# ebarnett2/batotp

Measured on AMD Instinct MI355X. Metric: constraint-evaluated waypoints/sec + traversal-time err vs CPU ref, higher is better.
Workload: dtype f64

## Files before the change

batotp_amd/csrc/batotp_hip.hip:

```cpp
#include <hip/hip_runtime.h>

#include <algorithm>
#include <cmath>
#include <cstdio>
#include <cstdlib>
#include <cstring>
#include <new>
#include <thread>
#include <type_traits>
#include <vector>

#include "batotp_hip.h"
#include "batotp_models.h"
#include "kernels.hip.h"
#include "sweep1.hip.h"
#include "sweep8.hip.h"
#include "pointwise_va.hip.h"
#include "spline_stream.hip.h"
#include "spline_tile.hip.h"
#include "spline_lanes.hip.h"
#include "resample.hip.h"
#include "output.hip.h"

static inline unsigned seriesBlock(int64_t series)
{
   const int64_t lanes = (series + 255) / 256;
   return (unsigned)(lanes < 4 ? 4 : (lanes > 64 ? 64 : lanes));
}

static inline bool seriesLanesPay(int64_t series) { return series <= 4096; }

using namespace bk;

constexpr int BATOTP_CERT_HOLD_DEFAULT = 3;

static thread_local char g_err[512] = "";

static int hipFail(hipError_t e, const char *what)
{
   snprintf(g_err, sizeof(g_err), "%s: %s", what, hipGetErrorString(e));
   return BATOTP_ERR_HIP;
}
#define HIP_TRY(call)                                              \
   do                                                              \
   {                                                               \
      hipError_t e_ = (call);                                      \
      if (e_ != hipSuccess) return hipFail(e_, #call);             \
   } while (0)

extern "C" const char *batotp_hip_last_error(void) { return g_err; }

#define BK_STR2(x) #x
#define BK_STR(x) BK_STR2(x)
static const char kBuiltWith[] = "clang " __clang_version__ " / HIP " BK_STR(HIP_VERSION_MAJOR) "." BK_STR(HIP_VERSION_MINOR) "." BK_STR(HIP_VERSION_PATCH);
static const char kFlatValidatedWith[] =
   "clang 22.0.0git (https://github.com/RadeonOpenCompute/llvm-project roc-7.2.0 26014 7b800a19466229b8479a78de19143dc33c3ab9b5) / HIP 7.2.26015";

extern "C" int batotp_hip_toolchain(char *built_with, char *validated_with, int32_t cap)
{
   if (cap < 1) return BATOTP_ERR_ARG;
   if (built_with) { strncpy(built_with, kBuiltWith, (size_t)cap - 1); built_with[cap - 1] = 0; }
   if (validated_with) { strncpy(validated_with, kFlatValidatedWith, (size_t)cap - 1); validated_with[cap - 1] = 0; }
   return BATOTP_OK;
}

struct Arena
{
   void *p = nullptr;
   size_t cap = 0;
};

struct batotp_ctx
{
   Arena ws[4];
   std::vector<double> kinTheta, kinTrig;
   Arena xfer;
   uint64_t rsEpoch = 0;
   int device = 0;
   hipStream_t stream = nullptr;
   hipStream_t stream2 = nullptr;
   hipEvent_t evJoin = nullptr;
   int overlap = 0;
   int sweepGroup = 0;
   int pathsPerWave = 0;
   int sweepTouch[2] = {-1, -1};
   int sweepHold[2] = {-2, -2};
   int splineTiles = -1;
   int flatForm = 1;
   int fastForward = 1;
   int certHold = -1;
   int poison = 0;
   int rsTrace = 0;
   uint64_t rsTraceSums[8] = {0, 0, 0, 0, 0, 0, 0, 0};
   unsigned long long *dTrace = nullptr;
   std::vector<double> rsTraceData[8];
   int64_t rsBudget = 0, outBudget = 0;
   int pathOrder = 1;
   int k3Form = 1;
   int flatStatus = 0;
   char builtWith[192] = "";
};

struct SweepPlan
{
   int feat = 0;
   bool uni = false;
   int lanes = 0;
   int ppw = 0;
   int hold = -1, touch = 0, ff = 0, holdc = 0;
   bool flat = false;
   bool form8 = false;
   int ff1 = 0;
};

struct batotp_batch
{
   batotp_ctx *ctx = nullptr;
   batotp_problem prob;
   DevProblem P;
   int32_t B = 0;
   int64_t cap = 0;
   int64_t totalKnots = 0;
   std::vector<PathInfo> pinfo;
   bool needPar = false;
   bool k3Pending = false;
   bool compact = false;
   bool pairsAll = false;
   int kmC = 0;
   bool kinDone = false, dynDone = false, sitesSet = false, revDone = false, trigSet = false;
   bool inPlace = false;
   bool revGone = false;
   bool mvcInCurves = false, mvcValid = false;
   bool revStale = false, fwdStale = false;

   DevProblem *dP = nullptr;
   PathInfo *dPinfo = nullptr;
   double *dY = nullptr, *dSC = nullptr, *dCoef = nullptr, *dSamp = nullptr, *dDyn = nullptr, *dTrig = nullptr, *dMvc = nullptr;
   double2 *dRev = nullptr, *dFwd = nullptr;
   batotp_path_result *dRes = nullptr;
   int *dOrder = nullptr;
   double *dProf = nullptr;
   double *dStage = nullptr;
   int *dSink = nullptr;
   double *dElim = nullptr;
   double *dKM = nullptr;
   batotp_serial_model *dModel = nullptr;
   batotp_serial_model hModel;
   double *dJTrig = nullptr;
   bool hasSerial = false, jtrigSet = false;
   int *dTileOff = nullptr, *dDirty = nullptr;
   double *dEdge = nullptr;
   int totalTiles = 0, nchMax = 0, lastTileNch = 0;
   double *dUp = nullptr;
   int64_t upDoubles = 0;
   int64_t maxN = 0;
   int64_t bytes = 0;

   hipEvent_t ev[5][2] = {};
   bool evValid[5] = {};
   SweepPlan lastPlan[2];
};

static int poisonFill(const batotp_ctx *ctx, void *p, size_t bytes, hipStream_t st)
{
   if (!ctx->poison || !p || !bytes) return BATOTP_OK;
   HIP_TRY(hipMemsetAsync(p, 0xFF, bytes, st));
   return BATOTP_OK;
}

static int devAlloc(batotp_batch *b, void **p, size_t bytes)
{
   if (bytes == 0) bytes = 8;
   hipError_t e = hipMalloc(p, bytes);
   if (e != hipSuccess)
   {
      hipFail(e, "hipMalloc");
      (void)hipGetLastError();
      return BATOTP_ERR_ALLOC;
   }
   b->bytes += (int64_t)bytes;
   if (b->ctx && b->ctx->poison)
   {
      e = hipMemsetAsync(*p, 0xFF, bytes, b->ctx->stream);
      if (e == hipSuccess) e = hipStreamSynchronize(b->ctx->stream);
      if (e != hipSuccess) return hipFail(e, "hipMemset (poison)");
   }
   return BATOTP_OK;
}

static int bind(batotp_ctx *ctx)
{
   HIP_TRY(hipSetDevice(ctx->device));
   return BATOTP_OK;
}

extern "C" int batotp_hip_device_count(int *count)
{
   if (!count) return BATOTP_ERR_ARG;
   int n = 0;
   hipError_t e = hipGetDeviceCount(&n);
   if (e != hipSuccess) { *count = 0; hipFail(e, "hipGetDeviceCount"); return BATOTP_ERR_NO_DEVICE; }
   *count = n;
   return BATOTP_OK;
}

static int uploadThomasTable()
{
   double tab[64];
   tab[0] = 0.0;
   double c = 1.0;
   c /= 4.0;
   tab[1] = c;
   int conv = -1;
   for (int i = 2; i < 64; ++i)
   {
      double ci = 1.0;
      ci /= 4.0 - 1.0 * tab[i - 1];
      tab[i] = ci;
      if (conv < 0 && tab[i] == tab[i - 1]) conv = i;
   }
   if (conv < 0 || conv > 60)
   {
      snprintf(g_err, sizeof(g_err), "Thomas coefficient table did not converge");
      return BATOTP_ERR_STATE;
   }
   double chk = 1.0;
   chk /= 4.0 - 1.0 * tab[63];
   if (chk != tab[63])
   {
      snprintf(g_err, sizeof(g_err), "Thomas coefficient table is not a fixed point");
      return BATOTP_ERR_STATE;
   }
   {
      const double den = 4.0 - 1.0 * tab[63];
      int e;
      const double m = frexp(den, &e);
      if (!(m < 1.0 - 1e-9))
      {
         snprintf(g_err, sizeof(g_err), "Thomas pivot unsuitable for the reciprocal divide");
         return BATOTP_ERR_STATE;
      }
      tab[0] = 1.0 / den;
   }
   HIP_TRY(hipMemcpyToSymbol(HIP_SYMBOL(c_ctab), tab, sizeof(tab)));
   double tcl[64];
   {
      double c0 = 1.0;
      c0 /= 2.0;
      tcl[0] = c0;
   }
   for (int i = 1; i < 64; ++i)
   {
      double ci = 1.0;
      ci /= 4.0 - 1.0 * tcl[i - 1];
      tcl[i] = ci;
   }
   {
      double chk2 = 1.0;
      chk2 /= 4.0 - 1.0 * tcl[63];
      if (chk2 != tcl[63] || tcl[62] != tcl[63])
      {
         snprintf(g_err, sizeof(g_err), "clamped Thomas coefficient table is not a fixed point");
         return BATOTP_ERR_STATE;
      }
   }
   HIP_TRY(hipMemcpyToSymbol(HIP_SYMBOL(c_ctab_cl), tcl, sizeof(tcl)));
   return BATOTP_OK;
}

extern "C" int batotp_hip_ctx_create(int device, batotp_ctx **out)
{
   if (!out) return BATOTP_ERR_ARG;
   *out = nullptr;
   int n = 0;
   hipError_t e = hipGetDeviceCount(&n);
   if (e != hipSuccess || n <= 0)
   {
      snprintf(g_err, sizeof(g_err), "no HIP device (%s)", e == hipSuccess ? "count = 0" : hipGetErrorString(e));
      return BATOTP_ERR_NO_DEVICE;
   }
   if (device < 0 || device >= n) return BATOTP_ERR_ARG;
   batotp_ctx *c = new (std::nothrow) batotp_ctx;
   if (!c) return BATOTP_ERR_ALLOC;
   c->device = device;
   strncpy(c->builtWith, kBuiltWith, sizeof(c->builtWith) - 1);
#ifdef BATOTP_TEST_HOOKS
   {
      const char *assume = getenv("BATOTP_ASSUME_TOOLCHAIN");
      if (assume && assume[0] && strcmp(assume, kFlatValidatedWith) != 0)
      {
         memset(c->builtWith, 0, sizeof(c->builtWith));
         strncpy(c->builtWith, assume, sizeof(c->builtWith) - 1);
      }
   }
#endif
   e = hipSetDevice(device);
   if (e != hipSuccess) { delete c; return hipFail(e, "hipSetDevice"); }
   e = hipStreamCreateWithFlags(&c->stream, hipStreamNonBlocking);
   if (e == hipSuccess) e = hipStreamCreateWithFlags(&c->stream2, hipStreamNonBlocking);
   if (e == hipSuccess) e = hipEventCreateWithFlags(&c->evJoin, hipEventDisableTiming);
   if (e != hipSuccess) { delete c; return hipFail(e, "hipStreamCreate"); }
   int rc = uploadThomasTable();
   if (rc != BATOTP_OK) { hipStreamDestroy(c->stream); delete c; return rc; }
   *out = c;
   return BATOTP_OK;
}

extern "C" int batotp_hip_ctx_destroy(batotp_ctx *ctx)
{
   if (!ctx) return BATOTP_OK;
   hipSetDevice(ctx->device);
   if (ctx->stream) hipStreamDestroy(ctx->stream);
   if (ctx->stream2) hipStreamDestroy(ctx->stream2);
   if (ctx->evJoin) hipEventDestroy(ctx->evJoin);
   for (Arena &a : ctx->ws)
      if (a.p) hipFree(a.p);
   if (ctx->xfer.p) hipFree(ctx->xfer.p);
   if (ctx->dTrace) hipFree(ctx->dTrace);
   delete ctx;
   return BATOTP_OK;
}

extern "C" int batotp_hip_ctx_trim(batotp_ctx *ctx)
{
   if (!ctx) return BATOTP_ERR_ARG;
   int rc = bind(ctx);
   if (rc) return rc;
   HIP_TRY(hipStreamSynchronize(ctx->stream));
   for (Arena &a : ctx->ws)
   {
      if (a.p) hipFree(a.p);
      a.p = nullptr; a.cap = 0;
   }
   if (ctx->xfer.p) { hipFree(ctx->xfer.p); ctx->xfer.p = nullptr; ctx->xfer.cap = 0; }
   ++ctx->rsEpoch;
   return BATOTP_OK;
}

extern "C" int batotp_hip_synchronize(batotp_ctx *ctx)
{
   if (!ctx) return BATOTP_ERR_ARG;
   int rc = bind(ctx);
   if (rc) return rc;
   HIP_TRY(hipStreamSynchronize(ctx->stream));
   HIP_TRY(hipStreamSynchronize(ctx->stream2));
   return BATOTP_OK;
}

extern "C" int batotp_hip_set_sweep_group(batotp_ctx *ctx, int32_t lanes)
{
   if (!ctx || !(lanes == 0 || lanes == 1 || lanes == 2 || lanes == 4 || lanes == 8 || lanes == 16 || lanes == 32 || lanes == 64)) return BATOTP_ERR_ARG;
   ctx->sweepGroup = lanes;
   return BATOTP_OK;
}

extern "C" int batotp_hip_set_overlap(batotp_ctx *ctx, int32_t on)
{
   if (!ctx) return BATOTP_ERR_ARG;
   ctx->overlap = on ? 1 : 0;
   return BATOTP_OK;
}

extern "C" int batotp_hip_set_sweep_hold(batotp_ctx *ctx, int32_t reverse, int32_t forward)
{
   if (!ctx || reverse < -2 || reverse > 8 || forward < -2 || forward > 8) return BATOTP_ERR_ARG;
   ctx->sweepHold[0] = reverse;
   ctx->sweepHold[1] = forward;
   return BATOTP_OK;
}

extern "C" int batotp_hip_set_flat_form(batotp_ctx *ctx, int32_t form)
{
   if (!ctx || form < 0 || form > 1) return BATOTP_ERR_ARG;
   ctx->flatForm = form;
   return BATOTP_OK;
}

extern "C" int batotp_hip_set_sweep_prefetch(batotp_ctx *ctx, int32_t reverse, int32_t forward)
{
   if (!ctx || reverse < -1 || reverse > 3 || forward < -1 || forward > 3) return BATOTP_ERR_ARG;
   ctx->sweepTouch[0] = reverse;
   ctx->sweepTouch[1] = forward;
   return BATOTP_OK;
}

extern "C" int batotp_hip_set_spline_tiles(batotp_ctx *ctx, int32_t on)
{
   if (!ctx) return BATOTP_ERR_ARG;
   ctx->splineTiles = on < 0 ? -1 : (on > 2 ? 2 : on);
   return BATOTP_OK;
}

extern "C" int batotp_hip_set_fast_forward(batotp_ctx *ctx, int32_t on)
{
   if (!ctx) return BATOTP_ERR_ARG;
   ctx->fastForward = on != 0 ? 1 : 0;
   return BATOTP_OK;
}

extern "C" int batotp_hip_set_resample_trace(batotp_ctx *ctx, int32_t on)
{
   if (!ctx) return BATOTP_ERR_ARG;
   ctx->rsTrace = on ? 1 : 0;
   return BATOTP_OK;
}

extern "C" int batotp_hip_set_poison(batotp_ctx *ctx, int32_t on)
{
   if (!ctx) return BATOTP_ERR_ARG;
   ctx->poison = on ? 1 : 0;
   return BATOTP_OK;
}

extern "C" int batotp_hip_set_cert_hold(batotp_ctx *ctx, int32_t hold)
{
   if (!ctx || hold < -1 || hold > 8) return BATOTP_ERR_ARG;
   ctx->certHold = hold;
   return BATOTP_OK;
}
static int certHoldOf(const batotp_ctx *ctx) { return ctx->certHold < 0 ? BATOTP_CERT_HOLD_DEFAULT : ctx->certHold; }
static int sweep8FastForward(const batotp_ctx *ctx) { return ctx->fastForward ? (1 | (certHoldOf(ctx) > 0 ? 2 : 0)) : 0; }

#ifdef S8_PROFILE
extern "C" int batotp_hip_debug_sweep8_counters(batotp_batch *b, double *out, int64_t n_doubles)
{
   if (!b || !out || n_doubles > (int64_t)b->B * 16 + 16) return BATOTP_ERR_ARG;
   HIP_TRY(hipStreamSynchronize(b->ctx->stream));
   HIP_TRY(hipMemcpy(out, b->dProf, sizeof(double) * (size_t)n_doubles, hipMemcpyDeviceToHost));
   return BATOTP_OK;
}
#endif

extern "C" int batotp_hip_set_path_order(batotp_ctx *ctx, int32_t mode)
{
   if (!ctx || (mode != 0 && mode != 1)) return BATOTP_ERR_ARG;
   ctx->pathOrder = mode;
   return BATOTP_OK;
}

extern "C" int batotp_hip_set_workspace_budget(batotp_ctx *ctx, int64_t resample_bytes, int64_t output_bytes)
{
   if (!ctx || resample_bytes < 0 || output_bytes < 0) return BATOTP_ERR_ARG;
   ctx->rsBudget = resample_bytes;
   ctx->outBudget = output_bytes;
   return BATOTP_OK;
}

extern "C" int batotp_hip_set_k3_form(batotp_ctx *ctx, int32_t form)
{
   if (!ctx || (form != 0 && form != 1)) return BATOTP_ERR_ARG;
   ctx->k3Form = form;
   return BATOTP_OK;
}

extern "C" int batotp_hip_spline_tile_fallbacks(batotp_batch *b, int32_t *series)
{
   if (!b || !series) return BATOTP_ERR_ARG;
   *series = 0;
   if (!b->totalTiles || b->lastTileNch == 0) return BATOTP_OK;
   int rc = bind(b->ctx);
   if (rc) return rc;
   std::vector<int> d((size_t)b->B * b->lastTileNch);
   HIP_TRY(hipMemcpy(d.data(), b->dDirty, sizeof(int) * d.size(), hipMemcpyDeviceToHost));
   int cnt = 0;
   for (int p = 0; p < b->B; ++p)
      if (b->pinfo[p].n >= ST_MIN_KNOTS)
         for (int c = 0; c < b->lastTileNch; ++c) cnt += d[(size_t)p * b->lastTileNch + c] ? 1 : 0;
   *series = cnt;
   return BATOTP_OK;
}

extern "C" int batotp_hip_set_paths_per_wave(batotp_ctx *ctx, int32_t n)
{
   if (!ctx || n < 0 || n > 64) return BATOTP_ERR_ARG;
   ctx->pathsPerWave = n;
   return BATOTP_OK;
}

extern "C" int batotp_hip_fp64_kat(batotp_ctx *ctx, int64_t n, const double *a, const double *b, double *q, double *r, double *p)
{
   if (!ctx || n <= 0 || !a || !b || !q || !r || !p) return BATOTP_ERR_ARG;
   int rc = bind(ctx);
   if (rc) return rc;
   double *d = nullptr;
   const size_t sz = sizeof(double) * (size_t)n;
   HIP_TRY(hipMalloc((void **)&d, 5 * sz));
   hipMemcpyAsync(d, a, sz, hipMemcpyHostToDevice, ctx->stream);
   hipMemcpyAsync(d + n, b, sz, hipMemcpyHostToDevice, ctx->stream);
   const int bs = 256;
   hipLaunchKernelGGL(k_kat, dim3((unsigned)((n + bs - 1) / bs)), dim3(bs), 0, ctx->stream, n, d, d + n, d + 2 * n, d + 3 * n, d + 4 * n);
   hipMemcpyAsync(q, d + 2 * n, sz, hipMemcpyDeviceToHost, ctx->stream);
   hipMemcpyAsync(r, d + 3 * n, sz, hipMemcpyDeviceToHost, ctx->stream);
   hipMemcpyAsync(p, d + 4 * n, sz, hipMemcpyDeviceToHost, ctx->stream);
   hipError_t e = hipStreamSynchronize(ctx->stream);
   hipFree(d);
   if (e != hipSuccess) return hipFail(e, "fp64_kat");
   return BATOTP_OK;
}

extern "C" int batotp_hip_div6_kat(batotp_ctx *ctx, int64_t n, const double *a, double *q)
{
   if (!ctx || n <= 0 || !a || !q) return BATOTP_ERR_ARG;
   int rc = bind(ctx);
   if (rc) return rc;
   double *d = nullptr;
   const size_t sz = sizeof(double) * (size_t)n;
   HIP_TRY(hipMalloc((void **)&d, 2 * sz));
   hipMemcpyAsync(d, a, sz, hipMemcpyHostToDevice, ctx->stream);
   hipLaunchKernelGGL(k_kat_div6, dim3((unsigned)((n + 255) / 256)), dim3(256), 0, ctx->stream, n, d, d + n);
   hipMemcpyAsync(q, d + n, sz, hipMemcpyDeviceToHost, ctx->stream);
   hipError_t e = hipStreamSynchronize(ctx->stream);
   hipFree(d);
   if (e != hipSuccess) return hipFail(e, "div6_kat");
   return BATOTP_OK;
}

extern "C" int batotp_hip_spline_lanes_kat(batotp_ctx *ctx, int64_t n, const double *y, double *sol, double *sol_seq, int32_t *redone)
{
   if (!ctx || n < 4 || n > (int64_t)1 << 30 || !y || !sol || !sol_seq || !redone) return BATOTP_ERR_ARG;
   int rc = bind(ctx);
   if (rc) return rc;
   double *d = nullptr;
   const size_t sz = sizeof(double) * (size_t)n;
   HIP_TRY(hipMalloc((void **)&d, 3 * sz + 64));
   double *dy = d, *dA = d + n, *dB = d + 2 * n;
   int64_t *dOff = reinterpret_cast<int64_t *>(d + 3 * n);
// ... 739 lines not shown
   std::vector<int64_t> nk(B);
   for (int p = 0; p < B; ++p) nk[p] = 12 + (p * 7) % 23;
   batotp_batch *b = nullptr;
   int rc = batotp_hip_batch_create(ctx, &prob, B, nk.data(), cap, &b);
   if (rc) return rc;
   std::vector<double> y, sres(B);
   uint64_t lcg = 0x9E3779B97F4A7C15ull;
   auto rnd = [&]() { lcg = lcg * 6364136223846793005ull + 1442695040888963407ull; return (double)(lcg >> 11) * (1.0 / 9007199254740992.0); };
   for (int p = 0; p < B; ++p)
   {
      const int64_t N = nk[p];
      sres[p] = 0.05 + 0.01 * (double)(p % 5);
      for (int j = 0; j < nJ; ++j)
      {
         const bool still = (j == 4 && p % 3 != 1) || (j == 5 && p % 3 != 2);
         const double c1 = 2.0 * rnd() - 1.0, c2 = 2.0 * rnd() - 1.0, c3 = 2.0 * rnd() - 1.0;
         for (int64_t i = 0; i < N; ++i)
         {
            const double x = (double)i / (double)(N - 1);
            y.push_back(still ? 0.25 : c1 * x + c2 * x * x * (1.0 - x) + c3 * x * x * x);
         }
      }
   }
   std::vector<batotp_path_result> rows[2];
   std::vector<double2> curves[2], curvesF[2];
   const int holdSaved[2] = {ctx->sweepHold[0], ctx->sweepHold[1]}, groupSaved = ctx->sweepGroup, ppwSaved = ctx->pathsPerWave;
   const int formSaved = ctx->flatForm, ffSaved = ctx->fastForward, certSaved = ctx->certHold;
   ctx->sweepGroup = 8; ctx->pathsPerWave = 8; ctx->flatForm = 1; ctx->fastForward = 1; ctx->certHold = -1;
   rc = batotp_hip_upload_knots(b, 0, B, y.data(), sres.data());
   if (!rc) rc = batotp_hip_precompute(b, 0);
   for (int form = 0; form < 2 && !rc; ++form)
   {
      ctx->sweepHold[0] = form == 0 ? -1 : 4;
      ctx->sweepHold[1] = form == 0 ? -1 : 8;
      rc = batotp_hip_sweep(b, -1);
      if (!rc) rc = batotp_hip_sweep(b, +1);
      rows[form].resize(B);
      if (!rc) rc = batotp_hip_get_results(b, rows[form].data());
      curves[form].resize((size_t)B * (size_t)cap);
      curvesF[form].resize((size_t)B * (size_t)cap);
      if (!rc && hipMemcpy(curves[form].data(), b->dRev, sizeof(double2) * curves[form].size(), hipMemcpyDeviceToHost) != hipSuccess) rc = BATOTP_ERR_HIP;
      if (!rc && hipMemcpy(curvesF[form].data(), b->dFwd, sizeof(double2) * curvesF[form].size(), hipMemcpyDeviceToHost) != hipSuccess) rc = BATOTP_ERR_HIP;
   }
   ctx->sweepHold[0] = holdSaved[0]; ctx->sweepHold[1] = holdSaved[1]; ctx->sweepGroup = groupSaved; ctx->pathsPerWave = ppwSaved;
   ctx->flatForm = formSaved; ctx->fastForward = ffSaved; ctx->certHold = certSaved;
   batotp_hip_batch_destroy(b);
   if (rc) return rc;
   bool eq = memcmp(rows[0].data(), rows[1].data(), sizeof(batotp_path_result) * (size_t)B) == 0;
   int finished = 0, stalled = 0;
   for (int p = 0; p < B && eq; ++p)
   {
      const int64_t n = rows[0][p].n_rev;
      if (n > 0) ++finished; else ++stalled;
      const size_t at = (size_t)p * (size_t)cap + (size_t)(cap - n);
      if (n > 0 && memcmp(&curves[0][at], &curves[1][at], sizeof(double2) * (size_t)n) != 0) eq = false;
      const int64_t nf = rows[0][p].n_fwd;
      const size_t atF = (size_t)p * (size_t)cap;
      if (nf > 0 && memcmp(&curvesF[0][atF], &curvesF[1][atF], sizeof(double2) * (size_t)nf) != 0) eq = false;
   }
   if (eq && (finished < 4 || stalled < 4))
   {
      snprintf(g_err, sizeof(g_err), "flat-loop canary degenerate: %d finished, %d stalled paths", finished, stalled);
      return BATOTP_ERR_STATE;
   }
   *same = eq;
   return BATOTP_OK;
}

static int flatLoopStatus(batotp_ctx *ctx)
{
   if (ctx->flatStatus != 0) return ctx->flatStatus;
   if (strcmp(ctx->builtWith, kFlatValidatedWith) != 0) return ctx->flatStatus = -1;
   ctx->flatStatus = -3;
   bool sameA = false, sameB = false;
   if (flatCanaryOnce(ctx, true, &sameA) != BATOTP_OK || flatCanaryOnce(ctx, false, &sameB) != BATOTP_OK) return ctx->flatStatus = -3;
   return ctx->flatStatus = (sameA && sameB) ? 1 : -2;
}

extern "C" int batotp_hip_flat_loop_status(batotp_ctx *ctx, int32_t *status)
{
   if (!ctx || !status) return BATOTP_ERR_ARG;
   int rc = bind(ctx);
   if (rc) return rc;
   *status = flatLoopStatus(ctx);
   return BATOTP_OK;
}

extern "C" int batotp_hip_last_sweep_launch(batotp_batch *b, int32_t dir, int32_t *lanes, int32_t *paths_per_wave, int32_t *hold)
{
   if (!b || (dir != 1 && dir != -1)) return BATOTP_ERR_ARG;
   const SweepPlan &p = b->lastPlan[dir == -1 ? 0 : 1];
   if (p.lanes == 0) return BATOTP_ERR_STATE;
   if (lanes) *lanes = p.lanes;
   if (paths_per_wave) *paths_per_wave = p.ppw;
   if (hold) *hold = p.flat ? p.hold : -1;
   return BATOTP_OK;
}

static SweepPlan planSweep(const batotp_batch *b, int dir)
{
   const batotp_ctx *ctx = b->ctx;
   const int k = dir == -1 ? 0 : 1;
   SweepPlan p;
   p.feat = featureLevel(b);
   p.uni = true;
   for (int i = 0; i < b->B; ++i) p.uni = p.uni && b->pinfo[i].uniform;
   const bool sweep1Applies = p.feat <= 2 && p.uni;

   int lanes = ctx->sweepGroup;
   if (lanes == 0)
   {
      lanes = (b->B <= (dir == -1 ? 2048 : 1024)) ? 32 : 8;
      if (sweep1Applies && b->B <= (dir == -1 ? 4608 : 3072)) lanes = 64;
      if (sweep1Applies && p.feat == -1 && b->B <= (dir == -1 ? 7600 : 5000)) lanes = 64;
   }
   if (b->pairsAll)
   {
      if (!sweep1Applies) return p;
      lanes = 64;
   }
   if (lanes == 64 && !sweep1Applies) lanes = 32;
   p.lanes = lanes;

   if (lanes == 64)
   {
      p.hold = -1; p.touch = 0; p.ff = ctx->fastForward; p.holdc = 0;
      const bool cableLines = p.feat == 2 && (b->P.flags & BATOTP_F_PARALLEL) != 0 && b->pairsAll;
      const int want = ctx->pathsPerWave;
      const bool compactVA = p.feat == -1;
      const bool two = (cableLines && (want == 2 || (want <= 0 && b->B > 2304))) ||
                       (compactVA && (want == 2 || (want <= 0 && b->B > (dir == -1 ? 3500 : 2304))));
      p.ppw = two ? 2 : 1;
      p.ff1 = (p.feat == 2 && (b->P.flags & BATOTP_F_PARALLEL) == 0) ? 1 : 0;
      return p;
   }

   const int maxPpw = 64 / lanes;
   int ppw = ctx->pathsPerWave;
   if (ppw <= 0)
   {
      ppw = (dir == -1) ? (b->B + 2047) / 2048 : (b->B + 1023) / 1024;
      if (dir == 1 && ppw > 4) ppw = std::max(4, (b->B + 2047) / 2048);
   }
   if (ppw < 1) ppw = 1;
   if (ppw > maxPpw) ppw = maxPpw;
   p.ppw = ppw;
   p.touch = (dir == -1) ? 1 : (ppw == 1 ? 3 : 0);
   p.ff = sweep8FastForward(ctx);
   p.holdc = std::max(1, certHoldOf(ctx));
   if (ctx->sweepTouch[k] >= 0) p.touch = ctx->sweepTouch[k];
   int hold = ctx->sweepHold[k];
   if (hold == -2)
   {
      const bool candidate = lanes == 8 && p.feat <= 0 && p.uni && ctx->flatForm == 1 && b->cap < ((int64_t)1 << 30);
      hold = -1;
      if (candidate && flatLoopStatus(b->ctx) == 1) hold = dir == -1 ? 4 : 8;
   }
   if (hold > 8) hold = 8;
   p.hold = hold;
   p.flat = (lanes == 8 || lanes == 4 || lanes == 2) && hold >= 0 && p.feat <= 0 && p.uni;
   p.form8 = p.flat && (lanes == 8 || lanes == 4) && ctx->flatForm == 1 && b->cap < ((int64_t)1 << 30);
   return p;
}

template <int G>
static void launchSweep(hipStream_t st, const SweepPlan &p, const SweepArgs &a)
{
   const unsigned waves = (unsigned)((a.B + p.ppw - 1) / p.ppw);
   const unsigned grid = (waves + (K4_BLOCK / 64) - 1) / (K4_BLOCK / 64);
   withFeature(p.feat, [&](auto f) {
      constexpr int F = decltype(f)::value;
      if (p.form8 && F <= 0)
      {
         constexpr int F8 = F <= 0 ? F : 0, G8 = G == 4 ? 4 : 8;
         if (a.dir == 1) hipLaunchKernelGGL((k_sweep8<G8, F8, 1>), dim3(grid), dim3(S8_BLOCK), 0, st, a);
         else hipLaunchKernelGGL((k_sweep8<G8, F8, -1>), dim3(grid), dim3(S8_BLOCK), 0, st, a);
      }
      else if (p.flat) hipLaunchKernelGGL((k_sweep<G, F, true, ((G == 8 || G == 4 || G == 2) && F <= 0)>), dim3(grid), dim3(K4_BLOCK), 0, st, a);
      else if (p.uni) hipLaunchKernelGGL((k_sweep<G, F, true>), dim3(grid), dim3(K4_BLOCK), 0, st, a);
      else hipLaunchKernelGGL((k_sweep<G, F, false>), dim3(grid), dim3(K4_BLOCK), 0, st, a);
   });
}

static void launchSweep1(hipStream_t st, const SweepPlan &p, const SweepArgs &a, bool pairsAll)
{
   const unsigned perBlock = (unsigned)(S1_BLOCK / 64) * (unsigned)p.ppw;
   const unsigned grid = ((unsigned)a.B + perBlock - 1) / perBlock;
   auto launch = [&](auto F, auto FF, auto PAIRS, auto NP) {
      if (a.dir == 1) hipLaunchKernelGGL((k_sweep1<F(), 1, FF(), PAIRS(), NP()>), dim3(grid), dim3(S1_BLOCK), 0, st, a);
      else hipLaunchKernelGGL((k_sweep1<F(), -1, FF(), PAIRS(), NP()>), dim3(grid), dim3(S1_BLOCK), 0, st, a);
   };
   auto onePath = [&](auto F, auto FF) {
      if (pairsAll) launch(F, FF, std::true_type(), Int<1>());
      else launch(F, FF, std::false_type(), Int<1>());
   };
   if (p.ppw == 2)
   {
      if (p.feat == 2) launch(Int<2>(), Int<0>(), std::true_type(), Int<2>());
      else launch(Int<-1>(), Int<0>(), std::false_type(), Int<2>());
   }
   else if (p.feat == 2 && p.ff1 == 0) onePath(Int<2>(), Int<0>());
   else if (p.feat == 2) onePath(Int<2>(), Int<1>());
   else if (p.feat == 1) onePath(Int<1>(), Int<0>());
   else if (p.feat == -1) launch(Int<-1>(), Int<0>(), std::false_type(), Int<1>());
   else onePath(Int<0>(), Int<0>());
}

extern "C" int batotp_hip_sweep(batotp_batch *b, int32_t dir)
{
   if (!b || (dir != 1 && dir != -1)) return BATOTP_ERR_ARG;
   int rc = readyForSweep(b);
   if (rc) return rc;
   if (dir == 1 && (!b->revDone || b->revGone)) return BATOTP_ERR_STATE;
   rc = bind(b->ctx);
   if (rc) return rc;
   b->mvcValid = false;
   SweepArgs a;
   a.P = b->P; a.dP = b->dP; a.pinfo = b->dPinfo; a.sC = b->dSC; a.coef = b->dCoef; a.km = b->compact ? b->dKM : nullptr;
   a.rev = b->dRev; a.fwd = b->dFwd; a.res = b->dRes; a.sink = b->dSink; a.prof = b->dMvc; a.cap = b->cap; a.B = b->B; a.dir = dir;
   a.order = b->ctx->pathOrder ? b->dOrder : nullptr;
#ifdef S8_PROFILE
   a.prof = b->dProf;
   hipMemsetAsync(b->dProf, 0, sizeof(double) * ((size_t)b->B * 16 + 16), b->ctx->stream);
#endif
   const int which = dir == -1 ? 3 : 4;
   const SweepPlan p = planSweep(b, dir);
   if (p.lanes == 0) { snprintf(g_err, sizeof(g_err), "pairs for all channels need uniform knot sites and constraints in serial form"); return BATOTP_ERR_STATE; }
   a.ppw = p.ppw; a.hold = p.hold; a.touch = p.touch; a.ff = p.ff; a.holdc = p.holdc;
   b->lastPlan[dir == -1 ? 0 : 1] = p;
   hipStream_t st = b->ctx->stream;
   evStart(b, which);
   switch (p.lanes)
   {
   case 64: launchSweep1(st, p, a, b->pairsAll); break;
   case 32: launchSweep<32>(st, p, a); break;
   case 1: launchSweep<1>(st, p, a); break;
   case 16: launchSweep<16>(st, p, a); break;
   case 4: launchSweep<4>(st, p, a); break;
   case 2: launchSweep<2>(st, p, a); break;
   default: launchSweep<8>(st, p, a); break;
   }
   evStop(b, which);
   HIP_TRY(hipGetLastError());
   HIP_TRY(hipStreamSynchronize(b->ctx->stream));
   if (dir == -1) { b->revDone = true; b->revGone = false; b->revStale = false; }
   else
   {
      b->fwdStale = false;
      if (b->inPlace) b->revGone = true;
   }
   return BATOTP_OK;
}

extern "C" int batotp_hip_optimize(batotp_batch *b)
{
   int rc = batotp_hip_precompute(b, 0);
   if (rc) return rc;
   rc = batotp_hip_sweep(b, -1);
   if (rc) return rc;
   return batotp_hip_sweep(b, 1);
}

extern "C" int batotp_hip_get_results(batotp_batch *b, batotp_path_result *out)
{
   if (!b || !out) return BATOTP_ERR_ARG;
   int rc = bind(b->ctx);
   if (rc) return rc;
   if ((rc = joinK3(b))) return rc;
   HIP_TRY(hipMemcpyAsync(out, b->dRes, sizeof(batotp_path_result) * b->B, hipMemcpyDeviceToHost, b->ctx->stream));
   HIP_TRY(hipStreamSynchronize(b->ctx->stream));
   return BATOTP_OK;
}

extern "C" int batotp_hip_download_curve(batotp_batch *b, int32_t path, int32_t which, double *s, double *sdot, int64_t cap, int64_t *n)
{
   if (!b || path < 0 || path >= b->B || (which != 1 && which != -1)) return BATOTP_ERR_ARG;
   if (which == -1 && b->revGone) return BATOTP_ERR_STATE;
   if (which == -1 ? b->revStale : b->fwdStale) return BATOTP_ERR_STATE;
   int rc = bind(b->ctx);
   if (rc) return rc;
   batotp_path_result r;
   HIP_TRY(hipMemcpy(&r, b->dRes + path, sizeof(r), hipMemcpyDeviceToHost));
   const int64_t avail = which == 1 ? r.n_fwd : r.n_rev;
   if (n) *n = avail;
   const int64_t m = avail < cap ? avail : cap;
   if (m <= 0 || (!s && !sdot)) return BATOTP_OK;
   const double2 *src = which == 1 ? b->dFwd + (int64_t)path * b->cap : b->dRev + (int64_t)path * b->cap + (b->cap - avail);
   double *tmp = nullptr;
   rc = xferReserve(b->ctx, sizeof(double) * 2 * (size_t)m, &tmp);
   if (rc) return rc;
   const int bs = 256;
   hipLaunchKernelGGL(k_curve_unpack, dim3((unsigned)((m + bs - 1) / bs)), dim3(bs), 0, b->ctx->stream, src, tmp, tmp + m, m);
   if (s) hipMemcpyAsync(s, tmp, sizeof(double) * (size_t)m, hipMemcpyDeviceToHost, b->ctx->stream);
   if (sdot) hipMemcpyAsync(sdot, tmp + m, sizeof(double) * (size_t)m, hipMemcpyDeviceToHost, b->ctx->stream);
   hipError_t e = hipStreamSynchronize(b->ctx->stream);
   if (e != hipSuccess) return hipFail(e, "download_curve");
   return BATOTP_OK;
}

extern "C" int batotp_hip_download_coeffs(batotp_batch *b, int32_t path, int32_t channel, double *c)
{
   if (!b || !c || path < 0 || path >= b->B) return BATOTP_ERR_ARG;
   const int dc = devChannel(b, channel);
   if (dc < 0) return BATOTP_ERR_ARG;
   int rc = bind(b->ctx);
   if (rc) return rc;
   const PathInfo &pi = b->pinfo[path];
   const int bs = 256;
   if (b->compact)
      hipLaunchKernelGGL(k_coef_from_sol, dim3((unsigned)((pi.n + bs - 1) / bs)), dim3(bs), 0, b->ctx->stream,
                         b->dKM + pi.koff * b->kmC * 2, b->kmC, dc, pi.n, b->dStage);
   else
      hipLaunchKernelGGL(k_coef_gather, dim3((unsigned)((pi.n + bs - 1) / bs)), dim3(bs), 0, b->ctx->stream,
                         b->dCoef + pi.koff * b->P.C * 4, b->P.C, dc, pi.n, b->dStage);
   HIP_TRY(hipMemcpyAsync(c, b->dStage, sizeof(double) * 4 * (size_t)pi.n, hipMemcpyDeviceToHost, b->ctx->stream));
   HIP_TRY(hipStreamSynchronize(b->ctx->stream));
   return BATOTP_OK;
}

extern "C" int batotp_hip_download_samples(batotp_batch *b, int32_t path, int32_t channel, double *out)
{
   if (!b || !out || path < 0 || path >= b->B || channel < 0 || channel >= b->P.Cin) return BATOTP_ERR_ARG;
   if (b->prob.flags & BATOTP_F_NO_SAMPLES) return BATOTP_ERR_STATE;
   int rc = bind(b->ctx);
   if (rc) return rc;
   const PathInfo &pi = b->pinfo[path];
   HIP_TRY(hipMemcpyAsync(out, b->dSamp + pi.koff * b->P.Cin * 3 + (int64_t)channel * 3 * pi.n, sizeof(double) * 3 * (size_t)pi.n,
                          hipMemcpyDeviceToHost, b->ctx->stream));
// ... 102 lines not shown
```

Baseline: 312.9 million.

## Add specialized locked forward sweep kernel for 8-lane flat form

Adds a dedicated forward-pass kernel for the 8-lane, hold-8, velocity/acceleration-only case that keeps stage state in registers, unrolls the six RK stages, buffers output points in shared memory and writes them in 4-point chunks. It is selected when flatForm is 1, the forward direction applies and hold is 8; a new flatForm value 2 keeps the older generic sweep8 path. The goal is to cut per-step generic overhead and scattered global stores in the forward sweep. In exchange it duplicates a large amount of sweep logic, which risks divergence from the reference path.

```diff
diff --git a/batotp_amd/csrc/batotp_hip.hip b/batotp_amd/csrc/batotp_hip.hip
--- a/batotp_amd/csrc/batotp_hip.hip
+++ b/batotp_amd/csrc/batotp_hip.hip
@@ -15,6 +15,7 @@
 #include "kernels.hip.h"
 #include "sweep1.hip.h"
 #include "sweep8.hip.h"
+#include "sweep8_fwd.hip.h"
 #include "pointwise_va.hip.h"
 #include "spline_stream.hip.h"
 #include "spline_tile.hip.h"
@@ -110,6 +111,7 @@
    int hold = -1, touch = 0, ff = 0, holdc = 0;
    bool flat = false;
    bool form8 = false;
+   bool lock = false;
    int ff1 = 0;
 };
 
@@ -371,7 +373,7 @@
 
 extern "C" int batotp_hip_set_flat_form(batotp_ctx *ctx, int32_t form)
 {
-   if (!ctx || form < 0 || form > 1) return BATOTP_ERR_ARG;
+   if (!ctx || form < 0 || form > 2) return BATOTP_ERR_ARG;
    ctx->flatForm = form;
    return BATOTP_OK;
 }
@@ -1417,14 +1419,15 @@
    int hold = ctx->sweepHold[k];
    if (hold == -2)
    {
-      const bool candidate = lanes == 8 && p.feat <= 0 && p.uni && ctx->flatForm == 1 && b->cap < ((int64_t)1 << 30);
+      const bool candidate = lanes == 8 && p.feat <= 0 && p.uni && ctx->flatForm != 0 && b->cap < ((int64_t)1 << 30);
       hold = -1;
       if (candidate && flatLoopStatus(b->ctx) == 1) hold = dir == -1 ? 4 : 8;
    }
    if (hold > 8) hold = 8;
    p.hold = hold;
    p.flat = (lanes == 8 || lanes == 4 || lanes == 2) && hold >= 0 && p.feat <= 0 && p.uni;
-   p.form8 = p.flat && (lanes == 8 || lanes == 4) && ctx->flatForm == 1 && b->cap < ((int64_t)1 << 30);
+   p.form8 = p.flat && (lanes == 8 || lanes == 4) && ctx->flatForm != 0 && b->cap < ((int64_t)1 << 30);
+   p.lock = p.form8 && lanes == 8 && dir == 1 && hold == 8 && ctx->flatForm == 1;
    return p;
 }
 
@@ -1438,7 +1441,8 @@
       if (p.form8 && F <= 0)
       {
          constexpr int F8 = F <= 0 ? F : 0, G8 = G == 4 ? 4 : 8;
-         if (a.dir == 1) hipLaunchKernelGGL((k_sweep8<G8, F8, 1>), dim3(grid), dim3(S8_BLOCK), 0, st, a);
+         if (p.lock) hipLaunchKernelGGL((k_sweep8_lock<F8>), dim3(grid), dim3(S8_BLOCK), 0, st, a);
+         else if (a.dir == 1) hipLaunchKernelGGL((k_sweep8<G8, F8, 1>), dim3(grid), dim3(S8_BLOCK), 0, st, a);
          else hipLaunchKernelGGL((k_sweep8<G8, F8, -1>), dim3(grid), dim3(S8_BLOCK), 0, st, a);
       }
       else if (p.flat) hipLaunchKernelGGL((k_sweep<G, F, true, ((G == 8 || G == 4 || G == 2) && F <= 0)>), dim3(grid), dim3(K4_BLOCK), 0, st, a);
diff --git a/batotp_amd/csrc/sweep8_fwd.hip.h b/batotp_amd/csrc/sweep8_fwd.hip.h
--- /dev/null
+++ b/batotp_amd/csrc/sweep8_fwd.hip.h
@@ -0,0 +1,449 @@
+#pragma once
+#include "sweep8.hip.h"
+#include <type_traits>
+
+namespace bk
+{
+
+template <int FEAT>
+__global__ void __launch_bounds__(S8_BLOCK, 2) k_sweep8_lock(SweepArgs a)
+{
+   static_assert(FEAT == -1 || FEAT == 0, "velocity / acceleration-only problems");
+   constexpr int G = 8, DIR = 1;
+   __shared__ double lim[6][8];
+   __shared__ double2 pts[S8_BLOCK / G][4];
+   const double rkB[6][6] = {{BK_B00, 0, 0, 0, 0, 0},
+                             {BK_B01, BK_B11, 0, 0, 0, 0},
+                             {BK_B02, BK_B12, BK_B22, 0, 0, 0},
+                             {BK_B03, BK_B13, BK_B23, BK_B33, 0, 0},
+                             {BK_B04, BK_B14, BK_B24, BK_B34, BK_B44, 0},
+                             {BK_B05, BK_B15, BK_B25, BK_B35, BK_B45, BK_B55}};
+   stage_limits(a.dP, lim);
+
+   const int lane = threadIdx.x & 63;
+   const int wave = blockIdx.x * (S8_BLOCK / 64) + (threadIdx.x >> 6);
+   const int j = lane % G;
+   const int slot = lane / G;
+   const int pslot = wave * a.ppw + slot;
+   if (slot >= a.ppw || pslot >= a.B) return;
+   const int p = a.order ? a.order[pslot] : pslot;
+   const bool writer = (j == 0);
+   const PathInfo pi = a.pinfo[p];
+   const int n = (int)pi.n;
+   const int64_t cap = a.cap;
+   double2 *mypts = pts[threadIdx.x / G];
+
+   Pt<G, FEAT, true> t;
+   pt_init(t, a.P, pi, a.sC, a.coef, a.km, lim, j, DIR);
+
+   double2 *out = a.fwd + (int64_t)p * cap;
+   batotp_path_result *__restrict__ r = a.res + p;
+   const int64_t nRev = r->n_rev;
+   if (nRev < 2)
+   {
+      if (writer) { r->n_fwd = 0; r->steps_fwd = 0; r->t_total = 0; r->status_fwd = r->status_rev | BATOTP_ST_CAPACITY; r->n_bisect_fail_fwd = 0; }
+      return;
+   }
+   const double2 *mvc = a.rev + (int64_t)p * cap + (cap - nRev);
+   const int nMvc = (int)nRev;
+   t.mvc = reinterpret_cast<const double *>(mvc);
+   t.nMvc = nMvc;
+   const int64_t revStart = (a.fwd == a.rev) ? cap - (int64_t)nMvc : ((int64_t)1 << 62);
+
+   const double absh = pi.integ_res;
+   const double h = absh;
+   const int64_t maxIntegSteps = (int64_t)floor(a.P.max_integ_time / pi.integ_res) + 1;
+   const double sres = pi.sres_c;
+   const double sEnd = sres * (double)(n - 1);
+   double s0v = 0.0;
+   double v0, w0 = 0;
+   t.segC = 0; t.tauC = 0; t.segMVC = 0; t.tauMVC = 0;
+   t.sCur = s0v;
+   t.sdotCur = 0;
+#pragma unroll 1
+   for (int pass = 0; pass < 2; ++pass)
+   {
+      accel_pt(t, j, w0);
+      if (pass == 0) { v0 = .1 * h * w0; t.sdotMin = v0; }
+      else v0 = t.sdotCur;
+      sdot_lim(t, j, v0);
+      if (pass == 0) { t.sdotMin = v0; t.sdotCur = v0; }
+   }
+   const double vBoot = v0;
+
+   const bool jOn = j < t.nJ;
+   const int jAt = jOn ? j : 0;
+   const double vmax = t.vmax[0], amax = t.amax[0];
+   double c1 = jOn ? t.rowTh[0].c1 : 0.0, c2x2 = jOn ? 2 * t.rowTh[0].c2 : 0.0;
+   double c3x3 = jOn ? 3 * t.rowTh[0].c3 : 0.0, c3x6 = jOn ? 6 * t.rowTh[0].c3 : 0.0;
+   double thD = t.thD[0], thD2 = t.thD2[0];
+   bool rOk = sdiv_window(thD);
+   double rD = sdiv_rcp(thD);
+   const bool accOn = (t.flags & BATOTP_F_JNT_ACC_ON) != 0;
+   const double thrV = t.thrV, thrA = t.thrA, vfact = t.vfact, afact = t.afact;
+   const double sdotCap = t.sdotCap, sddotMax = t.sddotMax, sdotMin = t.sdotMin;
+   const bool capOk = (sddotMax == sddotMax);
+   const int lastSeg = n - 2;
+   const int nIn = t.nIn;
+   const double2 *__restrict__ km = t.km;
+   const double *__restrict__ coef = t.coef;
+   const int rowStride = t.C * 4;
+   int seg = t.segC, rowSeg = t.rowSeg;
+   double2 kEdge = make_double2(0, 0), kPre = make_double2(0, 0);
+   int preIdx = -(1 << 20);
+   int segM = t.segMVC;
+   double mS0, mD0, mS1, mD1;
+   {
+      const double2 qa = mvc[segM], qb = mvc[segM + 1];
+      mS0 = qa.x; mD0 = qa.y; mS1 = qb.x; mD1 = qb.y;
+   }
+   unsigned status = t.status;
+   int nfail = t.nfail;
+   double sdotCur = t.sdotCur;
+   double sddotH = t.sddotH;
+
+   double v1 = 0, v2 = 0, v3 = 0, v4 = 0, v5 = 0;
+   double w1 = 0, w2 = 0, w3 = 0, w4 = 0, w5 = 0, w6 = 0;
+   double sCur = s0v;
+
+   const int iMax = (maxIntegSteps > 0x3ffffff0) ? 0x3ffffff0 : (int)maxIntegSteps;
+   const int capI = (int)cap;
+   const int revStartI = (revStart > 0x3fffffff) ? 0x3fffffff : (int)revStart;
+#define S8L_CURVE_FULL(i) ((i) >= capI || (i) + 64 >= revStartI + segM)
+
+   if (writer) { out[0] = make_double2(s0v, v0); mypts[0] = make_double2(s0v, v0); }
+
+   const double floorV = 0.0 / absh;
+   int i = 1;
+   unsigned endStatus = 0;
+   bool alive = true;
+   if (S8L_CURVE_FULL(i)) { endStatus = BATOTP_ST_CAPACITY; alive = false; }
+   double sN = 0, wN = 0;
+   double lowFact = .01, sdotGood = 0, sdotL = 0, sdotH = 0, sdotTry = 0;
+   int nGood = 0, nIter = 0;
+   bool stageFailed = false;
+#ifdef S8_PROFILE
+   double pc[16];
+   for (int k = 0; k < 16; ++k) pc[k] = 0;
+   const unsigned long long tLoop0 = __builtin_readcyclecounter();
+#endif
+
+   auto checkPass = [&](auto firstTag, bool &more) -> bool {
+      constexpr bool FIRST = decltype(firstTag)::value;
+      const double lowFact2 = lowFact * 2.0;
+      const double sdotLShrunk = dmax(.999 * 0.0, (1.0 - lowFact2) * sdotTry);
+      bool dec1, dec2;
+      const double num1 = fabs(sdotTry - sdotGood), num2 = sdotTry - sdotLShrunk;
+      bool close, tiny;
+      s8_ratio_lt_pair(num1, num2, sdotTry, close, dec1, tiny, dec2);
+      const double sdotSQ = sdotTry * sdotTry;
+      double H = sddotMax, L = -sddotMax;
+      bool force = false;
+      if (accOn)
+      {
+         const bool slow = fabs(thD) < thrV;
+         const double vTerm = thD2 * sdotSQ;
+         const double sa = (thD < 0.0) ? -amax : amax;
+         const double nH = sa - vTerm, nL = -sa - vTerm;
+         const bool fast = capOk & rOk & sdiv_window(nH) & sdiv_window(nL);
+         const double qH = sdiv_by(nH, thD, rD);
+         const double qL = sdiv_by(nL, thD, rD);
+         const bool use = jOn & !slow & fast;
+         const double Hm = vmin_f64(H, qH), Lm = vmax_f64(L, qL);
+         H = use ? Hm : H;
+         L = use ? Lm : L;
+         if (S8_RARE(jOn & (slow | !fast)))
+         {
+            S8_CNT(12, 1);
+            const int svpt = sgn(thD);
+            const double nHl = svpt * amax - vTerm, nLl = -svpt * amax - vTerm;
+            if (jOn && !slow && !fast)
+            {
+               H = dmin(H, nHl / thD);
+               L = dmax(L, nLl / thD);
+            }
+            if (jOn && slow && !(fabs(thD2) < thrA)) force |= sdotSQ > amax / fabs(thD2);
+         }
+      }
+      double Hred = force ? -kInf : H;
+      grp_min_max<G>(Hred, L);
+      sddotH = Hred;
+      const bool isViol = L > Hred;
+
+      const bool fin0 = !isViol && FIRST;
+      bool fin = fin0, failed = false;
+      more = false;
+      if (!FIRST || S8_ANY(!fin0))
+      {
+         const bool good = !isViol && !FIRST;
+         const bool shrink = isViol && nGood == 0;
+         if (S8_RARE((good & !dec1) | (shrink & !dec2)))
+         {
+            close = dec1 ? close : (num1 / sdotTry < .001);
+            tiny = dec2 ? tiny : (num2 / sdotTry < 1e-20);
+         }
+         const bool conv = good && (close || sdotTry < 0.0);
+         fin = fin0 || conv;
+         lowFact = shrink ? lowFact2 : lowFact;
+         sdotH = isViol ? sdotTry : sdotH;
+         sdotL = shrink ? sdotLShrunk : ((good && !conv) ? sdotTry : sdotL);
+         sdotGood = good ? sdotTry : sdotGood;
+         nGood += good ? 1 : 0;
+         sdotCur = conv ? sdotTry : sdotCur;
+         const bool collapsed = shrink && tiny;
+         failed = !fin && (nIter + 1 > 100 || sdotTry < 0.0 || collapsed);
+         nIter += fin ? 0 : 1;
+         sdotTry = (fin || failed) ? sdotTry : .5 * (sdotH + sdotL);
+         status |= failed ? (unsigned)BATOTP_ST_BISECT_FAIL : 0u;
+         nfail += failed ? 1 : 0;
+         stageFailed = failed;
+         if (FIRST && accOn)
+         {
+            const bool ffWant = ((a.ff & 1) != 0) && isViol && !failed;
+            if (S8_ANY(ffWant))
+            {
+               S8_CNT(11, 1);
+               if (ffWant)
+                  s8_certify(jOn, thD, thD2, rD, rOk, amax, thrV, thrA, sddotMax, lowFact, sdotH, sdotL, sdotTry, sdotGood, nGood, nIter);
+            }
+         }
+         if (FIRST) more = S8_ANY(!(fin || failed));
+      }
+      wN = fin ? sddotH : wN;
+      return fin || failed;
+   };
+
+   for (;;)
+   {
+      if (!S8_ANY(alive)) break;
+      if (alive)
+      {
+         sCur = s0v + h * v0;
+#include "sweep8_mvcwalk.inc"
+#pragma unroll
+         for (int st = 1; st <= 6; ++st)
+         {
+            S8_TICK(tA);
+            S8_CNT(1, 1); S8_CNT(2, __popcll(__ballot(1)) / G);
+            const double *bc = rkB[st - 1];
+            const double b0 = bc[0], b1 = bc[1], b2 = bc[2], b3 = bc[3], b4 = bc[4], b5 = bc[5];
+            double sdotT = 0, sddotT = 0;
+            sdotT += b0 * v0; sddotT += b0 * w0;
+            if (st > 1) { sdotT += b1 * v1; sddotT += b1 * w1; }
+            if (st > 2) { sdotT += b2 * v2; sddotT += b2 * w2; }
+            if (st > 3) { sdotT += b3 * v3; sddotT += b3 * w3; }
+            if (st > 4) { sdotT += b4 * v4; sddotT += b4 * w4; }
+            if (st > 5) { sdotT += b5 * v5; sddotT += b5 * w5; }
+            sN = s0v + h * sdotT;
+            double vN = v0 + h * sddotT;
+            vN = dmax(vN, floorV);
+            sCur = sN;
+
+            {
+#include "sweep8_mvcwalk.inc"
+               const double tauM = (sCur - mS0) / (mS1 - mS0);
+               const double sdotMVC = dmax(mD0 + tauM * (mD1 - mD0), sdotMin);
+               vN = (vN > sdotMVC) ? sdotMVC : vN;
+            }
+            vN = dmin(vN, sdotCap);
+            vN = dmax(vN, sdotMin);
+            {
+               double lim1 = kInf;
+               const bool on = jOn && fabs(thD) > thrV;
+               const bool fast = rOk & sdiv_window(vmax);
+               const double qv = fabs(sdiv_by(vmax, thD, rD));
+               lim1 = (on & fast) ? dmin(lim1, qv) : lim1;
+               if (S8_RARE(on & !fast))
+               {
+                  if (on && !fast) lim1 = dmin(lim1, fabs(vmax / thD));
+               }
+               lim1 = grp_min<G>(lim1);
+               vN = dmin(vN, lim1);
+            }
+            sdotCur = vN;
+            lowFact = .01; sdotGood = 0; nGood = 0; sdotL = 0; sdotH = vN; sdotTry = vN; nIter = 0; stageFailed = false;
+
+            double sSeg = sres * (double)seg, sNext = sres * (double)(seg + 1);
+            if (S8_ANY(!((sCur >= sSeg) & (sCur <= sNext))))
+            {
+               S8_CNT(10, 1);
+               for (;;)
+               {
+                  sSeg = sres * (double)seg;
+                  sNext = sres * (double)(seg + 1);
+                  const bool inside = (sCur >= sSeg) & (sCur <= sNext);
+                  const bool up = !inside & (sCur > sSeg), down = !inside & (sCur < sSeg);
+                  status |= (!inside & !up & !down) ? (unsigned)BATOTP_ST_NONFINITE : 0u;
+                  const bool mvUp = up & (seg < lastSeg), mvDn = down & (seg > 0);
+                  seg = mvUp ? seg + 1 : (mvDn ? seg - 1 : seg);
+                  if (!S8_ANY(mvUp | mvDn)) break;
+               }
+            }
+            const double tau = (sCur - sSeg) / (sNext - sSeg);
+            const bool chg = (seg != rowSeg);
+            if (S8_ANY(chg))
+            {
+               S8_CNT(9, 1);
+               if (chg)
+               {
+                  if (FEAT < 0)
+                  {
+                     const unsigned at = (unsigned)(seg * nIn + jAt);
+                     double yL = kEdge.x, solL = kEdge.y, yR = kPre.x, solR = kPre.y;
+                     bool literal = !(preIdx == seg + 1);
+                     const double xa = solR - solL, xb = solR + 2 * solL;
+                     literal |= !((fabs(xa) > 1e-280) & (fabs(xa) < 1e280) & (fabs(xb) > 1e-280) & (fabs(xb) < 1e280));
+                     double c3, sixthB;
+                     {
+                        const double qa = xa * (1.0 / 6.0), qb = xb * (1.0 / 6.0);
+                        c3 = __builtin_fma(__builtin_fma(-6.0, qa, xa), 1.0 / 6.0, qa);
+                        sixthB = __builtin_fma(__builtin_fma(-6.0, qb, xb), 1.0 / 6.0, qb);
+                     }
+                     if (S8_RARE(literal))
+                     {
+                        const bool hit = (preIdx == seg + 1);
+                        const double2 dl = km[at], dr = km[at + nIn];
+                        yL = hit ? yL : dl.x; solL = hit ? solL : dl.y;
+                        yR = hit ? yR : dr.x; solR = hit ? solR : dr.y;
+                        c3 = div6(solR - solL);
+                        sixthB = div6(solR + 2 * solL);
+                     }
+                     {
+                        kEdge = make_double2(yR, solR);
+                        int nxt = seg + 2;
+                        nxt = nxt < 0 ? 0 : (nxt > lastSeg + 1 ? lastSeg + 1 : nxt);
+                        kPre = km[(unsigned)(nxt * nIn + jAt)];
+                     }
+                     const double c2 = solL / 2.0;
+                     c1 = yR - yL - sixthB;
+                     c2x2 = 2 * c2; c3x3 = 3 * c3; c3x6 = 6 * c3;
+                     const int nxt = seg + 2;
+                     preIdx = nxt < 0 ? (-(1 << 20)) : (nxt > lastSeg + 1 ? (-(1 << 20)) : nxt);
+                  }
+                  else
+                  {
+                     const Coef4 k = *reinterpret_cast<const Coef4 *>(coef + (unsigned)(seg * rowStride) + jAt * 4);
+                     c1 = k.c1; c2x2 = 2 * k.c2; c3x3 = 3 * k.c3; c3x6 = 6 * k.c3;
+                  }
+                  rowSeg = seg;
+               }
+            }
+            {
+               const double tau2 = tau * tau;
+               thD = (c3x3 * tau2 + c2x2 * tau + c1) * vfact;
+               thD2 = (c3x6 * tau + c2x2) * afact;
+               rOk = sdiv_window(thD);
+               rD = sdiv_rcp(thD);
+            }
+            S8_TICK(tB);
+            S8_CYC(5, tA, tB);
+
+            S8_CNT(0, 1); S8_CNT(3, 1); S8_CNT(4, __popcll(__ballot(1)) / G); S8_CNT(13, __popcll(__ballot(1)) / G);
+            bool more;
+            bool ended = checkPass(std::true_type(), more);
+            while (more)
+            {
+               S8_CNT(0, 1); S8_CNT(3, 1); S8_CNT(4, __popcll(__ballot(!ended)) / G); S8_CNT(13, __popcll(__ballot(1)) / G);
+               if (!ended)
+               {
+                  bool unused;
+                  ended = checkPass(std::false_type(), unused);
+               }
+               more = S8_ANY(!ended);
+            }
+            S8_TICK(tC);
+            S8_CYC(6, tB, tC);
+
+            if (st == 1) { v1 = sdotCur; w1 = stageFailed ? w1 : wN; }
+            if (st == 2) { v2 = sdotCur; w2 = stageFailed ? w2 : wN; }
+            if (st == 3) { v3 = sdotCur; w3 = stageFailed ? w3 : wN; }
+            if (st == 4) { v4 = sdotCur; w4 = stageFailed ? w4 : wN; }
+            if (st == 5) { v5 = sdotCur; w5 = stageFailed ? w5 : wN; }
+         }
+         {
+            S8_CNT(8, 1);
+            const double vN = sdotCur;
+            const double wE = stageFailed ? w6 : wN;
+            s0v = sN; v0 = vN; w0 = wE; w6 = wE;
+            const int idx = i;
+            mypts[idx & 3] = make_double2(s0v, v0);
+            const bool fin = sCur > sres * (double)(lastSeg + 1);
+            const bool late = !fin && (i > iMax);
+            i = (fin || late) ? i : i + 1;
+            const bool full = !fin && !late && S8L_CURVE_FULL(i);
+            endStatus = late ? (unsigned)BATOTP_ST_MAX_INTEG_TIME : (full ? (unsigned)BATOTP_ST_CAPACITY : endStatus);
+            alive = !(fin || late || full);
+            const bool chunk = !fin && ((idx & 3) == 3);
+            if (chunk)
+            {
+               const int base = idx & ~3;
+               const int at = base + j;
+               if (j < 4 && at >= base && at <= idx) out[at] = mypts[j];
+            }
+         }
+      }
+   }
+#ifdef S8_PROFILE
+   pc[7] = (double)(__builtin_readcyclecounter() - tLoop0);
+   if (lane == 0 && a.prof)
+      for (int k = 0; k < 16; ++k) a.prof[(int64_t)wave * 16 + k] = pc[k];
+#endif
+
+   status |= endStatus;
+   if (endStatus != 0)
+   {
+      if (writer) { r->n_fwd = 0; r->steps_fwd = i; r->t_total = 0; r->status_fwd = status; r->n_bisect_fail_fwd = nfail; }
+      return;
+   }
+
+   const int nPts = i + 1;
+   double sCurPt = s0v, sdCurPt = v0;
+   const double2 qPrev = mypts[(nPts - 2) & 3];
+   const double sPrev = qPrev.x, sdPrev = qPrev.y;
+   const double sLast = sEnd;
+   {
+      const double sRat = (sLast - sPrev) / (sCurPt - sPrev);
+      sdCurPt = sdPrev + sRat * (sdCurPt - sdPrev);
+      sCurPt = sLast;
+      sdCurPt = mvc[nMvc - 1].y;
+   }
+   const double tElapsed = absh * (double)(nPts - 1);
+   int64_t nOut = nPts;
+
+   if (nPts >= 4)
+   {
+      const int idxLast = nPts - 1;
+      mypts[idxLast & 3] = make_double2(sCurPt, sdCurPt);
+      const int base = idxLast & ~3;
+      const int at = base + j;
+      if (j < 4 && at <= idxLast) out[at] = mypts[j];
+   }
+   else
+   {
+      status |= BATOTP_ST_SHORT; nOut = 4;
+      if (writer)
+      {
+         double ps[3], pd[3], tIn[3];
+         for (int k = 0; k < nPts; ++k)
+         {
+            const double2 q = (k == nPts - 1) ? make_double2(sCurPt, sdCurPt) : (k == 0 ? make_double2(0.0, vBoot) : make_double2(sPrev, sdPrev));
+            ps[k] = q.x; pd[k] = q.y;
+            tIn[k] = absh * (double)k;
+         }
+         const double tResNew = tIn[nPts - 1] / 3.;
+         int cur = 0;
+         for (int k = 0; k < 4; ++k)
+         {
+            const double tn = tResNew * (double)k;
+            while (!(tn < tIn[cur + 1] || cur == nPts - 2)) ++cur;
+            const double tauR = (tn - tIn[cur]) / (tIn[cur + 1] - tIn[cur]);
+            out[k] = make_double2(ps[cur] + (ps[cur + 1] - ps[cur]) * tauR, pd[cur] + (pd[cur + 1] - pd[cur]) * tauR);
+         }
+      }
+   }
+
+   if (writer) { r->n_fwd = nOut; r->steps_fwd = nPts - 1; r->t_total = tElapsed; r->status_fwd = status; r->n_bisect_fail_fwd = nfail; }
+}
+#undef S8L_CURVE_FULL
+
+}
```

Result: faster. 332.2 million, median of 6 (+6.2%).
